# evo-design/evo

Measured on AMD Instinct MI355X. Metric: nucleotides/sec forward scoring, evo-1 7B, higher is better.
Workload: dtype bf16; 1 GPU; evo-1-8k-base scoring, batch 8 x 8,192 nt per GPU (BASELINE configs[1]); batch_per_gpu=8, nt=8192, parallelism=single GPU

## Files before the change

### evo_amd/csrc/gemm.hip

```cpp
#include <stdlib.h>
#include "common.h"
#include "../../include/evo_mi355x.h"

#define GBM 256
#define GBN 256
#define GBK 64
#define G_ROW (GBK * 2)
#define G_SLAB (GBM * G_ROW)
#define G_NSLOT 5
#define G_NP 4

typedef uint32_t g_u32x4 __attribute__((ext_vector_type(4)));

#define G_VMCNT(N) asm volatile("s_waitcnt vmcnt(%0)" ::"n"(N) : "memory")
#define G_BARRIER() asm volatile("s_barrier" ::: "memory")

struct GemmArgs {
    const unsigned char* x; const unsigned char* w; const uint16_t* bias; const uint16_t* res; uint16_t* y;
    int64_t M; int N; int K;
    int tiles_n; int n_tiles; int tiles_m; int group_m;
    const float* rs = nullptr;
    float* ss = nullptr;
    int64_t ss_ld = 0;
    int64_t w_rows = 0;
    int tm_tiles = 0, row_skip = 0;
};

template <bool BIAS, bool RES>
__global__ __launch_bounds__(512, 1) void gemm_bf16_kernel(GemmArgs a) {
    __shared__ __attribute__((aligned(16))) unsigned char smem[G_NSLOT * G_SLAB];
    const int tid = threadIdx.x;
    const int lane = tid & 63;
    const int wave = __builtin_amdgcn_readfirstlane(tid >> 6);
    const int half = lane >> 5;
    const int l31 = lane & 31;
    const int wm = wave >> 2, wn = wave & 3;

    int tile;
    {
        const int bid = blockIdx.x, nt = a.n_tiles;
        const int q = nt >> 3, r = nt & 7, xcd = bid & 7, slot = bid >> 3;
        tile = (xcd < r ? xcd * (q + 1) : r * (q + 1) + (xcd - r) * q) + slot;
    }
    int tm, tn;
    {
        const int per_group = a.group_m * a.tiles_n;
        const int grp = tile / per_group, in_grp = tile - grp * per_group;
        const int first_m = grp * a.group_m;
        const int gsz = a.tiles_m - first_m < a.group_m ? a.tiles_m - first_m : a.group_m;
        tn = in_grp / gsz;
        tm = first_m + in_grp - tn * gsz;
    }
    const int64_t m0 = (int64_t)tm * GBM;
    const int n0 = tn * GBN;
    const int64_t kb = (int64_t)a.K * 2;
    const int nk = a.K / GBK;

    const unsigned char* srcx[G_NP];
    const unsigned char* srcw[G_NP];
#pragma unroll
    for (int jj = 0; jj < G_NP; ++jj) {
        const int pos = (wave + 8 * jj) * 1024 + 16 * lane;
        const int r = pos / G_ROW;
        const int col = ((((pos - r * G_ROW) >> 4) ^ (r >> 1)) & 7) * 16;
        int64_t m = m0 + r;
        if (m > a.M - 1) m = a.M - 1;
        srcx[jj] = a.x + m * kb + col;
        srcw[jj] = a.w + (int64_t)(n0 + r) * kb + col;
    }
    const uint32_t lds0 = (uint32_t)(uintptr_t)(__attribute__((address_space(3))) unsigned char*)smem;
    const uint32_t lds_dma = lds0 + wave * 1024;
#define G_DMA(SRC, H, JJ)                                                                                     \
    asm volatile("s_mov_b32 m0, %0\n\ts_nop 0\n\tglobal_load_lds_dwordx4 %1, off"                             \
                 ::"s"(lds_dma + ((H) % G_NSLOT) * G_SLAB + (JJ) * 8192),                                     \
                   "v"((SRC)[JJ] + (int64_t)(((H) >> 1) < nk ? ((H) >> 1) : nk - 1) * (GBK * 2)) : "memory", "m0")

    uint32_t x_rd[4], w_rd[4];
#pragma unroll
    for (int ks = 0; ks < 4; ++ks) {
        const int xr = wm * 128 + l31, wr = wn * 64 + l31;
        x_rd[ks] = lds0 + (uint32_t)(xr * G_ROW + (((2 * ks + half) ^ (xr >> 1)) & 7) * 16);
        w_rd[ks] = lds0 + (uint32_t)(wr * G_ROW + (((2 * ks + half) ^ (wr >> 1)) & 7) * 16);
    }

    f32x16_t acc[2][4];
#pragma unroll
    for (int i = 0; i < 2; ++i)
#pragma unroll
        for (int j = 0; j < 4; ++j)
#pragma unroll
            for (int r = 0; r < 16; ++r) acc[i][j][r] = 0.f;
    g_u32x4 wf[2][2], xf[2][4];

#define G_DSR(DST, ADDR, OFF) asm volatile("ds_read_b128 %0, %1 offset:%2" : "=v"(DST) : "v"(ADDR), "n"(OFF))
#define G_READ(XO, WO, KS, BUF)                                                                               \
    {                                                                                                         \
        const uint32_t wa_ = (WO) + w_rd[KS], xa_ = (XO) + x_rd[KS];                                          \
        G_DSR(wf[BUF][0], wa_, 0); G_DSR(wf[BUF][1], wa_, 32 * G_ROW);                                        \
        G_DSR(xf[BUF][0], xa_, 0); G_DSR(xf[BUF][1], xa_, 32 * G_ROW);                                        \
        G_DSR(xf[BUF][2], xa_, 64 * G_ROW); G_DSR(xf[BUF][3], xa_, 96 * G_ROW);                               \
    }
#define G_LGKM(N, BUF)                                                                                        \
    asm volatile("s_waitcnt lgkmcnt(%6)" : "+v"(wf[BUF][0]), "+v"(wf[BUF][1]), "+v"(xf[BUF][0]), "+v"(xf[BUF][1]), \
                 "+v"(xf[BUF][2]), "+v"(xf[BUF][3]) : "n"(N))
#define G_MFMA(I, J, BUF)                                                                                     \
    acc[I][J] = __builtin_amdgcn_mfma_f32_32x32x16_bf16(__builtin_bit_cast(bf16x8_t, wf[BUF][I]),             \
                                                        __builtin_bit_cast(bf16x8_t, xf[BUF][J]), acc[I][J], 0, 0, 0)
#define G_DMA_PIN(SRC, H, JJ)                                                                                 \
    {                                                                                                         \
        __builtin_amdgcn_sched_barrier(0);                                                                    \
        G_DMA(SRC, H, JJ);                                                                                    \
        __builtin_amdgcn_sched_barrier(0);                                                                    \
    }
#define G_MMA_DMA(BUF, SRC, H, JA, JB, JC, JD)                                                                \
    {                                                                                                         \
        G_MFMA(0, 0, BUF); G_MFMA(0, 1, BUF);                                                                 \
        if ((JA) >= 0) G_DMA_PIN(SRC, H, (JA) < 0 ? 0 : (JA));                                                    \
        G_MFMA(0, 2, BUF); G_MFMA(0, 3, BUF);                                                                 \
        if ((JB) >= 0) G_DMA_PIN(SRC, H, (JB) < 0 ? 0 : (JB));                                                    \
        G_MFMA(1, 0, BUF); G_MFMA(1, 1, BUF);                                                                 \
        if ((JC) >= 0) G_DMA_PIN(SRC, H, (JC) < 0 ? 0 : (JC));                                                    \
        G_MFMA(1, 2, BUF); G_MFMA(1, 3, BUF);                                                                 \
        if ((JD) >= 0) G_DMA_PIN(SRC, H, (JD) < 0 ? 0 : (JD));                                                    \
    }

#pragma unroll
    for (int jj = 0; jj < G_NP; ++jj) G_DMA(srcx, 0, jj);
#pragma unroll
    for (int jj = 0; jj < G_NP; ++jj) G_DMA(srcw, 1, jj);
    if (nk > 1) {
#pragma unroll
        for (int jj = 0; jj < G_NP; ++jj) G_DMA(srcx, 2, jj);
#pragma unroll
        for (int jj = 0; jj < G_NP; ++jj) G_DMA(srcw, 3, jj);
        G_VMCNT(2 * G_NP);
    } else {
        G_VMCNT(0);
    }
    G_BARRIER();
    G_READ(0, G_SLAB, 0, 0);
    for (int k = 0; k + 1 < nk; ++k) {
        const uint32_t xo = ((2 * k) % G_NSLOT) * G_SLAB, wo = ((2 * k + 1) % G_NSLOT) * G_SLAB;
        G_READ(xo, wo, 1, 1);
        G_LGKM(6, 0);
        __builtin_amdgcn_sched_barrier(0);
        G_MMA_DMA(0, srcx, 2 * k + 4, -1, 0, -1, 1);
        __builtin_amdgcn_sched_barrier(0);
        G_READ(xo, wo, 2, 0);
        G_LGKM(6, 1);
        __builtin_amdgcn_sched_barrier(0);
        G_MMA_DMA(1, srcx, 2 * k + 4, -1, 2, -1, 3);
        __builtin_amdgcn_sched_barrier(0);
        G_READ(xo, wo, 3, 1);
        G_LGKM(6, 0);
        __builtin_amdgcn_sched_barrier(0);
        G_MMA_DMA(0, srcx, 0, -1, -1, -1, -1);
        __builtin_amdgcn_sched_barrier(0);
        G_LGKM(0, 1);
        G_VMCNT(G_NP);
        G_BARRIER();
        G_READ(((2 * k + 2) % G_NSLOT) * G_SLAB, ((2 * k + 3) % G_NSLOT) * G_SLAB, 0, 0);
        __builtin_amdgcn_sched_barrier(0);
        G_MMA_DMA(1, srcw, 2 * k + 5, 0, 1, 2, 3);
        __builtin_amdgcn_sched_barrier(0);
    }
    {
        const int k = nk - 1;
        const uint32_t xo = ((2 * k) % G_NSLOT) * G_SLAB, wo = ((2 * k + 1) % G_NSLOT) * G_SLAB;
        G_READ(xo, wo, 1, 1);
        G_LGKM(6, 0);
        G_MMA_DMA(0, srcx, 0, -1, -1, -1, -1);
        G_READ(xo, wo, 2, 0);
        G_LGKM(6, 1);
        G_MMA_DMA(1, srcx, 0, -1, -1, -1, -1);
        G_READ(xo, wo, 3, 1);
        G_LGKM(6, 0);
        G_MMA_DMA(0, srcx, 0, -1, -1, -1, -1);
        G_LGKM(0, 1);
        G_MMA_DMA(1, srcx, 0, -1, -1, -1, -1);
        G_VMCNT(0);
    }

    G_BARRIER();
    {
        constexpr int PITCH = 144;
        unsigned char* tr = smem + wave * (128 * PITCH);
        const int rsub = lane >> 3, cseg = lane & 7;
        const int nseg = n0 + wn * 64 + cseg * 8;
        if (RES) {
#pragma unroll 4
            for (int it = 0; it < 16; ++it) {
                const int row = it * 8 + rsub;
                const int64_t m = m0 + wm * 128 + row;
                uint4 r = make_uint4(0, 0, 0, 0);
                if (m < a.M) r = *(const uint4*)(a.res + m * a.N + nseg);
                *(uint4*)(tr + row * PITCH + cseg * 16) = r;
            }
        }
        asm volatile("" ::: "memory");
        uint2 bpk[2][4];
        if (BIAS) {
#pragma unroll
            for (int i = 0; i < 2; ++i)
#pragma unroll
                for (int g = 0; g < 4; ++g) bpk[i][g] = *(const uint2*)(a.bias + n0 + wn * 64 + i * 32 + 8 * g + 4 * half);
        }
#pragma unroll
        for (int j = 0; j < 4; ++j)
#pragma unroll
            for (int i = 0; i < 2; ++i)
#pragma unroll
                for (int g = 0; g < 4; ++g) {
                    unsigned char* cell = tr + (j * 32 + l31) * PITCH + (i * 32 + 8 * g + 4 * half) * 2;
                    float v[4] = {acc[i][j][4 * g], acc[i][j][4 * g + 1], acc[i][j][4 * g + 2], acc[i][j][4 * g + 3]};
                    if (BIAS) {
                        v[0] += bf_lo(bpk[i][g].x); v[1] += bf_hi(bpk[i][g].x);
                        v[2] += bf_lo(bpk[i][g].y); v[3] += bf_hi(bpk[i][g].y);
                    }
                    if (RES) {
                        const uint2 r = *(const uint2*)cell;
                        v[0] += bf_lo(r.x); v[1] += bf_hi(r.x); v[2] += bf_lo(r.y); v[3] += bf_hi(r.y);
                    }
                    uint2 o;
                    o.x = pack_bf2(v[0], v[1]);
                    o.y = pack_bf2(v[2], v[3]);
                    *(uint2*)cell = o;
                }
        asm volatile("" ::: "memory");
#pragma unroll 4
        for (int it = 0; it < 16; ++it) {
            const int row = it * 8 + rsub;
            const int64_t m = m0 + wm * 128 + row;
            const uint4 o = *(const uint4*)(tr + row * PITCH + cseg * 16);
            if (m < a.M) *(uint4*)(a.y + m * a.N + nseg) = o;
        }
    }
}


#ifndef GR_DGAP
#define GR_DGAP 8
#endif
#ifndef GE_ORDER
#define GE_ORDER 1
#endif
#ifndef GE_FULL
#define GE_FULL 1
#endif
static_assert(!GE_FULL || GE_ORDER == 1, "GE_FULL pairs the strips of GE_ORDER 1");
#if GE_ORDER == 0
#define GE_B(U) ((U) >> 3)
#define GE_J(U) ((U) & 7)
#else
#define GE_B(U) ((U) & 3)
#define GE_J(U) ((U) >> 2)
#endif

#ifndef GE_STPOL_ID
#define GE_STPOL_ID 0
#endif
#if GE_STPOL_ID == 1
#define GE_STPOL " nt"
#elif GE_STPOL_ID == 2
#define GE_STPOL " sc1"
#elif GE_STPOL_ID == 3
#define GE_STPOL " sc0 sc1"
#else
#define GE_STPOL ""
#endif
#ifndef GR_MIDB
#define GR_MIDB 1
#endif
#ifndef GR_PAD
#define GR_PAD 0
#endif
#ifndef GR_ALIGN
#define GR_ALIGN 0
#endif
#ifndef GR_PROFILE
#define GR_PROFILE 0
#endif

template <bool BIAS, bool RES, int MODE, bool XB = false, int NF = 0>
__global__ __launch_bounds__(256, 1) void gemmr_bf16_kernel(GemmArgs a) {
    constexpr bool STATS = (NF & 1) != 0, SCALE = (NF & 2) != 0;
    static_assert(!STATS || (RES && MODE == 0), "the statistic rides on the launches that write the residual stream");
    static_assert(!SCALE || !RES, "the row factor belongs to the launches that read the normalised stream");
    constexpr uint32_t XSTEP = XB ? 16384u : (uint32_t)(GBK * 2);
    __shared__ __attribute__((aligned(16))) unsigned char smem[G_NSLOT * G_SLAB];
    const int tid = threadIdx.x;
    const int lane = tid & 63;
    const int wave = __builtin_amdgcn_readfirstlane(tid >> 6);
    const int wm = wave >> 1, wn = wave & 1;
    const uint32_t kb = (uint32_t)a.K * 2;
    const int nk = a.K / GBK;

    int t_first, t_step, n_my;
    {
        const int bid = blockIdx.x, per = gridDim.x >> 3;
        const int xcd = bid & 7, slot = bid >> 3;
        const int q = a.n_tiles >> 3, r = a.n_tiles & 7;
        const int xs = xcd < r ? xcd * (q + 1) : r * (q + 1) + (xcd - r) * q;
        const int xn = q + (xcd < r ? 1 : 0);
        t_first = xs + slot;
        t_step = per;
        n_my = slot < xn ? (xn - slot + per - 1) / per : 0;
    }
    if (n_my == 0) return;
    auto tile_origin = [&](int tile, int64_t& m0, int& n0) {
        if constexpr (MODE == 3) {
            const int per_group = a.group_m * a.tiles_m;
            const int grp = tile / per_group, in_grp = tile - grp * per_group;
            const int first_n = grp * a.group_m;
            const int gsz = a.tiles_n - first_n < a.group_m ? a.tiles_n - first_n : a.group_m;
            const int tm = in_grp / gsz;
            m0 = (int64_t)tm * GBM;
            n0 = (first_n + in_grp - tm * gsz) * GBN;
            return;
        }
        const int per_group = a.group_m * a.tiles_n;
        const int grp = tile / per_group, in_grp = tile - grp * per_group;
        const int first_m = grp * a.group_m;
        const int gsz = a.tiles_m - first_m < a.group_m ? a.tiles_m - first_m : a.group_m;
        const int tn = in_grp / gsz;
        m0 = (int64_t)(first_m + in_grp - tn * gsz) * GBM;
        n0 = tn * GBN;
    };

    auto src_row = [&](int n0) -> uint32_t {
        if constexpr (MODE == 3 && SCALE) return (uint32_t)n0 + (uint32_t)((n0 / GBN) / a.tm_tiles) * (uint32_t)a.row_skip;
        else return (uint32_t)n0;
    };

    const int r0 = 8 * wave + (lane >> 3);
    const uint32_t xs_ = (uint32_t)(((lane & 7) ^ r0) & 7);
    const uint32_t voff0 = XB ? (uint32_t)r0 * 32u + (xs_ >> 1) * 4096u + (xs_ & 1) * 16u
                              : (uint32_t)r0 * kb + xs_ * 16;
    const uint32_t row32 = 32u * kb;
    uint32_t voff[8], wvoff[8];
    const int wrow = 8 * ((r0 >> 2) & 3) + 4 * ((r0 >> 4) & 1) + (r0 & 3);
    const uint32_t wvoff0 = (uint32_t)wrow * kb + (uint32_t)((((lane & 7) ^ r0) & 7) * 16);
#pragma unroll
    for (int jj = 0; jj < 8; ++jj) {
        voff[jj] = XB ? voff0 + (uint32_t)(jj & 3) * 1024u + (uint32_t)(jj >> 2) * 128u * kb : voff0 + jj * row32;
        wvoff[jj] = wvoff0 + jj * row32;
    }
    const uint64_t xa64 = (uint64_t)a.x, wa64 = (uint64_t)a.w;
    const g_u32x4 rx = {(uint32_t)xa64, (uint32_t)(xa64 >> 32) & 0xffffu,
                        (uint32_t)((XB ? (a.M + 127) / 128 * 128 : a.M) * (int64_t)kb), 0x00020000u};
    const g_u32x4 rw = {(uint32_t)wa64, (uint32_t)(wa64 >> 32) & 0xffffu, (uint32_t)((MODE == 3 && SCALE ? a.w_rows : (int64_t)a.N) * kb), 0x00020000u};
    const uint32_t lds0 = (uint32_t)(uintptr_t)(__attribute__((address_space(3))) unsigned char*)smem;
    const uint32_t lds_dma = lds0 + wave * 1024;

    int f_i = 0, f_k = 0;
    uint32_t fxs, fws;
    {
        int64_t m0; int n0;
        tile_origin(t_first, m0, n0);
        fxs = (uint32_t)(m0 * kb);
        fws = src_row(n0) * kb;
    }
    auto fetch_advance = [&]() {
        if (f_k + 1 < nk) { ++f_k; fxs += XSTEP; fws += GBK * 2; }
        else if (f_i + 1 < n_my) {
            ++f_i; f_k = 0;
            int64_t m0; int n0;
            tile_origin(t_first + f_i * t_step, m0, n0);
            fxs = (uint32_t)(m0 * kb);
            fws = src_row(n0) * kb;
        }
    };
    uint32_t nx0 = 0, nw0 = 0, nfxs = 0, nfws = 0, fxp = 0, fwp = 0;
    int f_rem = 0;
    auto next_tile_origin = [&]() {
        if (f_i + 1 < n_my) {
            int64_t m0; int n0;
            tile_origin(t_first + (f_i + 1) * t_step, m0, n0);
            nx0 = (uint32_t)(m0 * kb);
            nw0 = src_row(n0) * kb;
        }
    };
#define GD_M0(V) asm volatile("s_mov_b32 m0, %0" ::"s"(V) : "memory", "m0")
#ifndef GR_ABL
#define GR_ABL 0
#endif
#define GD_DMAX(JJ) asm volatile("buffer_load_dwordx4 %0, %1, %2 offen lds" ::"v"(voff[JJ]), "s"(rx), "s"(fxs) : "memory")
#define GD_DMAW(JJ) asm volatile("buffer_load_dwordx4 %0, %1, %2 offen lds" ::"v"(wvoff[JJ]), "s"(rw), "s"(fws) : "memory")

    const int l15 = lane & 15, lq = lane >> 4;
    uint32_t x_rd[2], w_rd[2];
#pragma unroll
    for (int kh = 0; kh < 2; ++kh) {
        const int xr = wm * 128 + l15, wr = wn * 128 + l15;
        x_rd[kh] = lds0 + (uint32_t)(xr * G_ROW + (((4 * kh + lq) ^ xr) & 7) * 16);
        w_rd[kh] = lds0 + (uint32_t)(wr * G_ROW + (((4 * kh + lq) ^ wr) & 7) * 16);
    }

    const int ldy = MODE == 3 ? GBN : a.N;
    const uint32_t ep_voff = (uint32_t)((wm * 128 + l15) * ldy + wn * 128 + 8 * lq) * 2u;
    const int ep_rows16 = 16 * ldy * 2;
    const uint32_t ep_voff_f = (uint32_t)((wm * 128 + (l15 & 7)) * ldy + wn * 128 + 8 * lq + 32 * (l15 >> 3)) * 2u;
    const uint32_t ep_boff = (uint32_t)(wn * 128 + 8 * lq) * 2u;
    const uint32_t ep_rboff = (uint32_t)(wm * 128 + l15) * 2u;
    const uint32_t ep_rsoff = (uint32_t)(wm * 128 + l15) * 4u;
    const uint32_t ep_rsoff3 = (uint32_t)(wn * 128 + 8 * lq) * 4u;
    const int ep_gn = a.N >> 1;
    const uint32_t ep_voff_g = (uint32_t)((wm * 128 + (l15 & 7)) * ep_gn + wn * 64 + 8 * lq + 32 * (l15 >> 3)) * 2u;
    const int ep_grows16 = 16 * ep_gn * 2;
    f32x4_t acc[8][8];
#define GR_ZERO1(I, J) { _Pragma("unroll") for (int r_ = 0; r_ < 4; ++r_) acc[I][J][r_] = 0.f; asm volatile("" : "+a"(acc[I][J])); }
#define GR_ZERO() _Pragma("unroll") for (int i = 0; i < 8; ++i) _Pragma("unroll") for (int j = 0; j < 8; ++j) GR_ZERO1(i, j)
    GR_ZERO();
    asm volatile("s_nop 7" ::: "memory");
    g_u32x4 wf[2][8], xf[2][8];

#define GR_LGKM(N, BUF)                                                                                       \
    asm volatile("s_waitcnt lgkmcnt(%16)" : "+v"(wf[BUF][0]), "+v"(wf[BUF][1]), "+v"(wf[BUF][2]), "+v"(wf[BUF][3]), \
                 "+v"(wf[BUF][4]), "+v"(wf[BUF][5]), "+v"(wf[BUF][6]), "+v"(wf[BUF][7]),                      \
                 "+v"(xf[BUF][0]), "+v"(xf[BUF][1]), "+v"(xf[BUF][2]), "+v"(xf[BUF][3]),                      \
                 "+v"(xf[BUF][4]), "+v"(xf[BUF][5]), "+v"(xf[BUF][6]), "+v"(xf[BUF][7]) : "n"(N))
#define GR_MFMA(I, J, BUF)                                                                                    \
    asm volatile("v_mfma_f32_16x16x32_bf16 %0, %1, %2, %0" : "+a"(acc[I][J]) : "v"(wf[BUF][I]), "v"(xf[BUF][J]))
#define GR_RD1(XO, WO, KH, BUF, Q)                                                                            \
    { if ((Q) < 8) G_DSR(xf[BUF][(Q) & 7], (XO) + x_rd[KH], ((Q) & 7) * 16 * G_ROW);                          \
      else G_DSR(wf[BUF][(Q) & 7], (WO) + w_rd[KH], ((Q) & 7) * 16 * G_ROW); }
#define GR_GAP(G, RXO, RWO, RKH, RBUF)                                                                        \
    {                                                                                                         \
        __builtin_amdgcn_sched_barrier(0);                                                                    \
        constexpr int g_ = (G), s_ = g_ & 63;                                                                 \
         \
         \
        if constexpr (g_ == 64 && GR_MIDB) { G_VMCNT(8); if (!(GR_ABL & 2)) G_BARRIER(); }                    \
        if constexpr ((s_ & 1) == 0 && s_ < 32 && !(GR_ABL & 8)) { GR_RD1(RXO, RWO, RKH, RBUF, s_ >> 1); }    \
        if constexpr (g_ < 64 && s_ < 8 * GR_DGAP && (s_ % GR_DGAP) == 1 && !(GR_ABL & 16)) GD_M0(fxl + (s_ / GR_DGAP) * 4096);        \
        if constexpr (g_ < 64 && s_ < 8 * GR_DGAP && (s_ % GR_DGAP) == GR_DGAP / 2 + 1 && !(GR_ABL & 1)) GD_DMAX(s_ / GR_DGAP);       \
        if constexpr (g_ >= 64 && s_ < 8 * GR_DGAP && (s_ % GR_DGAP) == 1 && !(GR_ABL & 16)) GD_M0(fwl + (s_ / GR_DGAP) * 4096);       \
        if constexpr (g_ >= 64 && s_ < 8 * GR_DGAP && (s_ % GR_DGAP) == GR_DGAP / 2 + 1 && !(GR_ABL & 1)) GD_DMAW(s_ / GR_DGAP);      \
         \
         \
        if constexpr (g_ == 67) { fxp = fxs + XSTEP; fwp = fws + GBK * 2; GS_PIN2(fxp, fwp); }              \
        if constexpr (g_ == 71) { f_rem -= 1; GS_PIN1(f_rem); }                                               \
        if constexpr (g_ == 75) { nfxs = f_rem == 0 ? nx0 : fxp; GS_PIN1(nfxs); }                             \
        if constexpr (g_ == 87) { nfws = f_rem == 0 ? nw0 : fwp; GS_PIN1(nfws); }                             \
        if constexpr (g_ == 110) { c_k -= 1; GS_PIN1(c_k); }                                                  \
        if constexpr (g_ == 91) { const bool z_ = f_rem == 0; f_rem = z_ ? nk : f_rem; f_i += z_ ? 1 : 0; GS_PIN2(f_rem, f_i); } \
        if constexpr (g_ == 83) { fxs = nfxs; GS_PIN1(fxs); }                                                 \
         \
        if constexpr (g_ == 96) { r_t0 = xo; xo = nxo; GS_PIN2(r_t0, xo); }                                   \
        if constexpr (g_ == 98) { r_t1 = wo; wo = nwo; GS_PIN2(r_t1, wo); }                                   \
        if constexpr (g_ == 100) { nxo = fxo; nwo = r_t0; GS_PIN2(nxo, nwo); }                                \
        if constexpr (g_ == 102) { fxo = r_t1; fxl = lds_dma + r_t1; GS_PIN2(fxo, fxl); }                     \
        if constexpr (g_ == 126) { fws = nfws; fwl = lds_dma + xo; GS_PIN2(fws, fwl); }                       \
        __builtin_amdgcn_sched_barrier(0);                                                                    \
    }
#define GR_ROW8(SS, I, BUF, RXO, RWO, RKH, RBUF)                                                              \
    {                                                                                                         \
        GR_MFMA(I, 0, BUF); GR_GAP(64 * (SS) + 8 * (I) + 0, RXO, RWO, RKH, RBUF); GR_MFMA(I, 1, BUF); GR_GAP(64 * (SS) + 8 * (I) + 1, RXO, RWO, RKH, RBUF); \
        GR_MFMA(I, 2, BUF); GR_GAP(64 * (SS) + 8 * (I) + 2, RXO, RWO, RKH, RBUF); GR_MFMA(I, 3, BUF); GR_GAP(64 * (SS) + 8 * (I) + 3, RXO, RWO, RKH, RBUF); \
        GR_MFMA(I, 4, BUF); GR_GAP(64 * (SS) + 8 * (I) + 4, RXO, RWO, RKH, RBUF); GR_MFMA(I, 5, BUF); GR_GAP(64 * (SS) + 8 * (I) + 5, RXO, RWO, RKH, RBUF); \
        GR_MFMA(I, 6, BUF); GR_GAP(64 * (SS) + 8 * (I) + 6, RXO, RWO, RKH, RBUF); GR_MFMA(I, 7, BUF); GR_GAP(64 * (SS) + 8 * (I) + 7, RXO, RWO, RKH, RBUF); \
    }
#define GR_SUB(SS, BUF, RXO, RWO, RKH, RBUF)                                                                  \
    {                                                                                                         \
        GR_ROW8(SS, 0, BUF, RXO, RWO, RKH, RBUF); GR_ROW8(SS, 1, BUF, RXO, RWO, RKH, RBUF);                   \
        GR_ROW8(SS, 2, BUF, RXO, RWO, RKH, RBUF); GR_ROW8(SS, 3, BUF, RXO, RWO, RKH, RBUF);                   \
        GR_ROW8(SS, 4, BUF, RXO, RWO, RKH, RBUF); GR_ROW8(SS, 5, BUF, RXO, RWO, RKH, RBUF);                   \
        GR_ROW8(SS, 6, BUF, RXO, RWO, RKH, RBUF); GR_ROW8(SS, 7, BUF, RXO, RWO, RKH, RBUF);                   \
    }
#define GS_PIN1(A) asm volatile("" : "+s"(A))
#define GS_PIN2(A, B) asm volatile("" : "+s"(A), "+s"(B))

#pragma unroll
    for (int jj = 0; jj < 8; ++jj) { GD_M0(lds_dma + 0 * G_SLAB + jj * 4096); asm volatile("s_nop 0"); GD_DMAX(jj); }
#pragma unroll
    for (int jj = 0; jj < 8; ++jj) { GD_M0(lds_dma + 1 * G_SLAB + jj * 4096); asm volatile("s_nop 0"); GD_DMAW(jj); }
    fetch_advance();
#pragma unroll
    for (int jj = 0; jj < 8; ++jj) { GD_M0(lds_dma + 2 * G_SLAB + jj * 4096); asm volatile("s_nop 0"); GD_DMAX(jj); }
#pragma unroll
    for (int jj = 0; jj < 8; ++jj) { GD_M0(lds_dma + 3 * G_SLAB + jj * 4096); asm volatile("s_nop 0"); GD_DMAW(jj); }
    fetch_advance();
    f_rem = nk - f_k;
    next_tile_origin();
    G_VMCNT(16);
    G_BARRIER();
    {
        const uint32_t x0_ = 0, w0_ = G_SLAB;
#pragma unroll
        for (int q = 0; q < 16; ++q) GR_RD1(x0_, w0_, 0, 0, q);
    }

#if GR_PROFILE
    const bool prof = blockIdx.x == 0 && wave == 0;
    uint64_t tp[12] = {0, 0, 0, 0, 0, 0, 0, 0, 0, 0, 0, 0}, tl = __builtin_readcyclecounter();
#define GR_STAMP(K) if (prof) { const uint64_t n_ = __builtin_readcyclecounter(); tp[K] += n_ - tl; tl = n_; }
#else
#define GR_STAMP(K)
#endif
    uint32_t xo = 0, wo = G_SLAB, nxo = 2 * G_SLAB, nwo = 3 * G_SLAB, fxo = 4 * G_SLAB;
    uint32_t fxl = lds_dma + 4 * G_SLAB, fwl = lds_dma, r_t0 = 0, r_t1 = 0;
#if GR_PAD
    asm volatile(".rept %0\n\ts_nop 0\n\t.endr" :: "n"(GR_PAD));
#endif
#if GR_ALIGN
    asm volatile(".p2align %0" :: "n"(GR_ALIGN));
#endif
    for (int c_i = 0; c_i < n_my; ++c_i) {
#define GR_KSTEP()                                                                                            \
        {                                                                                                     \
            GR_LGKM(0, 0);                                                                                    \
            GR_STAMP(5);                                                                                      \
            GR_SUB(0, 0, xo, wo, 1, 1);                                                                       \
            GR_STAMP(0);                                                                                      \
            GR_LGKM(0, 1);                                        \
            GR_STAMP(1);                                                                                      \
            if (!GR_MIDB) { G_VMCNT(8); GR_STAMP(2); if (!(GR_ABL & 2)) G_BARRIER(); }                        \
            GR_STAMP(6);                                                                                      \
            GR_SUB(1, 1, nxo, nwo, 0, 0);                                                                     \
            GR_STAMP(3);                                                                                      \
        }
        for (int c_k = nk; c_k != 0;) GR_KSTEP();
        {
            asm volatile("s_nop 7\n\ts_nop 7" ::: "memory");
            int64_t m0; int n0;
            tile_origin(t_first + c_i * t_step, m0, n0);
            GR_STAMP(7);
            if constexpr (MODE == 1) {
                const int rows_ok = a.M - m0 < GBM ? (int)(a.M - m0) : GBM;
                const uint64_t y64 = (uint64_t)(a.y + m0 * ep_gn);
                const g_u32x4 yd = {(uint32_t)y64, (uint32_t)(y64 >> 32) & 0xffffu, (uint32_t)(rows_ok * ep_gn * 2), 0x00020000u};
                g_u32x4 ost[8], gq[2];
                float rsj[8];
                if constexpr (SCALE) {
#pragma unroll
                    for (int j = 0; j < 8; ++j)
                        asm volatile("global_load_dword %0, %1, %2" : "=v"(rsj[j]) : "v"(ep_rsoff), "s"(a.rs + m0 + 16 * j) : "memory");
                    asm volatile("s_waitcnt vmcnt(0)" : "+v"(rsj[0]), "+v"(rsj[1]), "+v"(rsj[2]), "+v"(rsj[3]), "+v"(rsj[4]), "+v"(rsj[5]),
                                 "+v"(rsj[6]), "+v"(rsj[7]) :: "memory");
                }
#pragma unroll
                for (int j = 0; j < 8; ++j) {
#pragma unroll
                    for (int pp = 0; pp < 2; ++pp) {
                        __builtin_amdgcn_sched_barrier(0);
                        float z1[8], z2[8];
#pragma unroll
                        for (int r = 0; r < 4; ++r) {
                            asm volatile("v_accvgpr_read_b32 %0, %1" : "=v"(z1[r]) : "a"(acc[4 * pp][j][r]));
                            asm volatile("v_accvgpr_read_b32 %0, %1" : "=v"(z1[4 + r]) : "a"(acc[4 * pp + 1][j][r]));
                            asm volatile("v_accvgpr_read_b32 %0, %1" : "=v"(z2[r]) : "a"(acc[4 * pp + 2][j][r]));
                            asm volatile("v_accvgpr_read_b32 %0, %1" : "=v"(z2[4 + r]) : "a"(acc[4 * pp + 3][j][r]));
                        }
                        GR_ZERO1(4 * pp, j); GR_ZERO1(4 * pp + 1, j); GR_ZERO1(4 * pp + 2, j); GR_ZERO1(4 * pp + 3, j);
                        if constexpr (SCALE) {
#pragma unroll
                            for (int e = 0; e < 8; ++e) { z1[e] *= rsj[j]; z2[e] *= rsj[j]; }
                        }
#pragma unroll
                        for (int e = 0; e < 8; e += 2) {
                            const uint32_t u1 = pack_bf2(z1[e], z1[e + 1]), u2 = pack_bf2(z2[e], z2[e + 1]);
                            const f32x2_t uu = {bf_lo(u1), bf_hi(u1)}, ww = {bf_lo(u2), bf_hi(u2)};
                            const f32x2_t oo = gelu_gate2(uu, ww);
                            gq[pp][e >> 1] = pack_bf2(oo[0], oo[1]);
                        }
                    }
                    const bool low = l15 < 8;
                    g_u32x4 &s1 = ost[(2 * j) & 7], &s2 = ost[(2 * j + 1) & 7];
#pragma unroll
                    for (int d = 0; d < 4; ++d) {
                        const uint32_t give = low ? gq[1][d] : gq[0][d];
                        const uint32_t recv = (uint32_t)__builtin_amdgcn_update_dpp(0, (int)give, 0x128, 0xf, 0xf, false);
                        s1[d] = low ? gq[0][d] : recv;
                        s2[d] = low ? recv : gq[1][d];
                    }
                    const int so = n0 + j * ep_grows16;
                    asm volatile("buffer_store_dwordx4 %0, %1, %2, %3 offen" GE_STPOL :: "v"(s1), "v"(ep_voff_g), "s"(yd), "s"(so) : "memory");
                    asm volatile("buffer_store_dwordx4 %0, %1, %2, %3 offen" GE_STPOL :: "v"(s2), "v"(ep_voff_g), "s"(yd), "s"(so + ep_grows16 / 2) : "memory");
                    if (j >= 3) { asm volatile("" :: "v"(ost[(2 * j + 2) & 7])); asm volatile("" :: "v"(ost[(2 * j + 3) & 7])); }
                }
                __builtin_amdgcn_sched_barrier(0);
#pragma unroll
                for (int k = 0; k < 8; ++k) asm volatile("" :: "v"(ost[k]));
                GR_STAMP(8);
            } else {
            const int rows_ok = a.M - m0 < GBM ? (int)(a.M - m0) : GBM;
            const uint64_t y64 = (uint64_t)(MODE == 3 ? a.y + ((int64_t)(n0 / GBN) * a.M + m0) * GBN : a.y + m0 * a.N);
            const uint64_t r64 = (uint64_t)((RES ? a.res : a.y) + m0 * a.N);
            const g_u32x4 yd = {(uint32_t)y64, (uint32_t)(y64 >> 32) & 0xffffu, (uint32_t)(rows_ok * ldy * 2), 0x00020000u};
            const g_u32x4 rd = {(uint32_t)r64, (uint32_t)(r64 >> 32) & 0xffffu, RES ? (uint32_t)(rows_ok * a.N * 2) : 0u, 0x00020000u};
#define GE_SOFF(U) ((MODE == 3 ? 0 : n0 * 2) + 64 * GE_B(U) + GE_J(U) * ep_rows16)
#define GE_NR 6
#define GE_LOAD(U) asm volatile("buffer_load_dwordx4 %0, %1, %2, %3 offen" : "=v"(rr[(U) % GE_NR]) : "v"(ep_voff), "s"(rd), "s"(GE_SOFF(U)) : "memory")
            g_u32x4 rr[GE_NR], bq[4], ost[8], o_even;
            uint32_t rbq[8];
            float rsj[8];
            g_u32x4 rsq[4][2];
            if constexpr (SCALE && MODE == 0) {
#pragma unroll
                for (int j = 0; j < 8; ++j)
                    asm volatile("global_load_dword %0, %1, %2" : "=v"(rsj[j]) : "v"(ep_rsoff), "s"(a.rs + m0 + 16 * j) : "memory");
                asm volatile("s_waitcnt vmcnt(0)" : "+v"(rsj[0]), "+v"(rsj[1]), "+v"(rsj[2]), "+v"(rsj[3]), "+v"(rsj[4]), "+v"(rsj[5]),
                             "+v"(rsj[6]), "+v"(rsj[7]) :: "memory");
            }
            if constexpr (SCALE && MODE == 3) {
                const float* rs0 = a.rs + src_row(n0);
#pragma unroll
                for (int b = 0; b < 4; ++b) {
                    asm volatile("global_load_dwordx4 %0, %1, %2" : "=v"(rsq[b][0]) : "v"(ep_rsoff3), "s"(rs0 + b * 32) : "memory");
                    asm volatile("global_load_dwordx4 %0, %1, %2" : "=v"(rsq[b][1]) : "v"(ep_rsoff3), "s"(rs0 + b * 32 + 4) : "memory");
                }
                asm volatile("s_waitcnt vmcnt(0)" : "+v"(rsq[0][0]), "+v"(rsq[0][1]), "+v"(rsq[1][0]), "+v"(rsq[1][1]), "+v"(rsq[2][0]),
                             "+v"(rsq[2][1]), "+v"(rsq[3][0]), "+v"(rsq[3][1]) :: "memory");
            }
            float ssq = 0.f, sst[4];
            if (BIAS && MODE != 3) {
#pragma unroll
                for (int b = 0; b < 4; ++b)
                    asm volatile("global_load_dwordx4 %0, %1, %2" : "=v"(bq[b]) : "v"(ep_boff), "s"(a.bias + n0 + b * 32) : "memory");
            }
            if (BIAS && MODE == 3) {
#pragma unroll
                for (int j = 0; j < 8; ++j)
                    asm volatile("global_load_ushort %0, %1, %2" : "=v"(rbq[j]) : "v"(ep_rboff), "s"(a.bias + m0 + 16 * j) : "memory");
                asm volatile("s_waitcnt vmcnt(0)" : "+v"(rbq[0]), "+v"(rbq[1]), "+v"(rbq[2]), "+v"(rbq[3]), "+v"(rbq[4]), "+v"(rbq[5]),
                             "+v"(rbq[6]), "+v"(rbq[7]) :: "memory");
            }
            if (RES) {
#pragma unroll
                for (int u = 0; u < GE_NR; ++u) GE_LOAD(u);
            }
            if (BIAS && !RES && MODE != 3) asm volatile("s_waitcnt vmcnt(0)" : "+v"(bq[0]), "+v"(bq[1]), "+v"(bq[2]), "+v"(bq[3]) :: "memory");
#pragma unroll
            for (int u = 0; u < 32; ++u) {
                const int b = GE_B(u), j = GE_J(u);
                __builtin_amdgcn_sched_barrier(0);
                if (RES) {
                    if (u + GE_NR <= 32) asm volatile("s_waitcnt vmcnt(%5)" : "+v"(rr[u % GE_NR]), "+v"(bq[0]), "+v"(bq[1]), "+v"(bq[2]), "+v"(bq[3]) : "n"(GE_NR - 1) : "memory");
                    else asm volatile("s_waitcnt vmcnt(0)" : "+v"(rr[u % GE_NR]) :: "memory");
                }
                float v[8];
#pragma unroll
                for (int r = 0; r < 4; ++r) {
                    asm volatile("v_accvgpr_read_b32 %0, %1" : "=v"(v[r]) : "a"(acc[2 * b][j][r]));
                    asm volatile("v_accvgpr_read_b32 %0, %1" : "=v"(v[4 + r]) : "a"(acc[2 * b + 1][j][r]));
                }
                GR_ZERO1(2 * b, j); GR_ZERO1(2 * b + 1, j);
                if constexpr (SCALE && MODE == 0) {
#pragma unroll
                    for (int e = 0; e < 8; ++e) v[e] *= rsj[j];
                }
                if constexpr (SCALE && MODE == 3) {
#pragma unroll
                    for (int e = 0; e < 8; ++e) v[e] *= __uint_as_float(rsq[b][e >> 2][e & 3]);
                }
                if (BIAS && MODE != 3) {
                    v[0] += bf_lo(bq[b][0]); v[1] += bf_hi(bq[b][0]); v[2] += bf_lo(bq[b][1]); v[3] += bf_hi(bq[b][1]);
                    v[4] += bf_lo(bq[b][2]); v[5] += bf_hi(bq[b][2]); v[6] += bf_lo(bq[b][3]); v[7] += bf_hi(bq[b][3]);
                }
                if (BIAS && MODE == 3) {
                    const float rb = bf_lo(rbq[j]);
#pragma unroll
                    for (int e = 0; e < 8; ++e) v[e] += rb;
                }
                if (RES) {
                    const g_u32x4 r = rr[u % GE_NR];
                    v[0] += bf_lo(r[0]); v[1] += bf_hi(r[0]); v[2] += bf_lo(r[1]); v[3] += bf_hi(r[1]);
                    v[4] += bf_lo(r[2]); v[5] += bf_hi(r[2]); v[6] += bf_lo(r[3]); v[7] += bf_hi(r[3]);
                }
                g_u32x4 o;
                o[0] = pack_bf2(v[0], v[1]); o[1] = pack_bf2(v[2], v[3]); o[2] = pack_bf2(v[4], v[5]); o[3] = pack_bf2(v[6], v[7]);
                if constexpr (STATS) {
                    static_assert(GE_ORDER == 1, "the statistic closes an m tile at b == 3");
#pragma unroll
                    for (int d = 0; d < 4; ++d) {
                        const float lo_ = bf_lo(o[d]), hi_ = bf_hi(o[d]);
                        ssq = fmaf(lo_, lo_, ssq);
                        ssq = fmaf(hi_, hi_, ssq);
                    }
                    if (b == 3) {
                        float t_ = ssq + __uint_as_float((uint32_t)__builtin_amdgcn_ds_swizzle((int)__float_as_uint(ssq), 0x401f));
                        t_ += __shfl_xor(t_, 32);
                        sst[j & 3] = t_;
                        const float* sp_ = a.ss + ((int64_t)(n0 / 128 + wn) * a.ss_ld + m0 + 16 * j);
                        asm volatile("global_store_dword %0, %1, %2" :: "v"(ep_rsoff), "v"(sst[j & 3]), "s"(sp_) : "memory");
                        ssq = 0.f;
                    }
                }
#if GE_FULL
                if ((u & 1) == 0) o_even = o;
                else {
                    const bool low = l15 < 8;
                    g_u32x4 &s1 = ost[(u - 1) & 7], &s2 = ost[u & 7];
#pragma unroll
                    for (int d = 0; d < 4; ++d) {
                        const uint32_t give = low ? o[d] : o_even[d];
                        const uint32_t recv = (uint32_t)__builtin_amdgcn_update_dpp(0, (int)give, 0x128, 0xf, 0xf, false);
                        s1[d] = low ? o_even[d] : recv;
                        s2[d] = low ? recv : o[d];
                    }
                    asm volatile("buffer_store_dwordx4 %0, %1, %2, %3 offen" GE_STPOL :: "v"(s1), "v"(ep_voff_f), "s"(yd), "s"(GE_SOFF(u - 1)) : "memory");
                    asm volatile("buffer_store_dwordx4 %0, %1, %2, %3 offen" GE_STPOL :: "v"(s2), "v"(ep_voff_f), "s"(yd), "s"(GE_SOFF(u - 1) + ep_rows16 / 2) : "memory");
                    if (u >= 7) { asm volatile("" :: "v"(ost[(u + 1) & 7])); asm volatile("" :: "v"(ost[(u + 2) & 7])); }
                }
#else
                ost[u & 7] = o;
                asm volatile("buffer_store_dwordx4 %0, %1, %2, %3 offen" GE_STPOL :: "v"(ost[u & 7]), "v"(ep_voff), "s"(yd), "s"(GE_SOFF(u)) : "memory");
                if (u >= 7) asm volatile("" :: "v"(ost[(u + 1) & 7]));
#endif
                if (RES && u + GE_NR < 32) GE_LOAD(u + GE_NR);
            }
            __builtin_amdgcn_sched_barrier(0);
#pragma unroll
            for (int k = 0; k < 8; ++k) asm volatile("" :: "v"(ost[k]));
            if constexpr (STATS) asm volatile("" :: "v"(sst[0]), "v"(sst[1]), "v"(sst[2]), "v"(sst[3]));
            GR_STAMP(8);
#undef GE_LOAD
#undef GE_NR
#undef GE_SOFF
            }
            next_tile_origin();
            GR_STAMP(9);
            asm volatile("s_nop 7" ::: "memory");
            GR_STAMP(4);
        }
    }
    G_VMCNT(0);
#if GR_PROFILE
    if (prof && lane == 0) {
        for (int k = 0; k < 12; ++k) ((float*)a.y)[k] = (float)tp[k];
        ((float*)a.y)[12] = (float)(n_my * nk);
        ((float*)a.y)[13] = (float)n_my;
    }
#endif
}

extern "C" int evo_linear_mfma_bf16(const void* x, const void* w, const void* bias, const void* residual, void* y,
                                    int64_t M, int64_t N, int64_t K, void* stream) {
    return evo_linear_mfma_nf_bf16(x, w, bias, residual, y, nullptr, nullptr, 0, M, N, K, stream);
}

extern "C" int evo_linear_mfma_nf_bf16(const void* x, const void* w, const void* bias, const void* residual, void* y,
                                       const float* row_scale, float* sumsq, int64_t ss_ld, int64_t M, int64_t N, int64_t K, void* stream) {
    if (M <= 0 || N <= 0 || K <= 0 || N % GBN != 0 || K % GBK != 0 || N > 0x7fffffff / 2) return -1;
    if ((row_scale && (residual || sumsq)) || (sumsq && (!residual || ss_ld < (M + GBM - 1) / GBM * GBM))) return -1;
    if ((row_scale || sumsq) && !(K >= 2 * GBK && M * K * 2 < 0xffffffffll && N * K * 2 < 0xffffffffll)) return -1;
    GemmArgs a;
    a.rs = row_scale; a.ss = sumsq; a.ss_ld = ss_ld;
    a.x = (const unsigned char*)x; a.w = (const unsigned char*)w; a.bias = (const uint16_t*)bias;
    a.res = (const uint16_t*)residual; a.y = (uint16_t*)y;
    a.M = M; a.N = (int)N; a.K = (int)K;
    a.tiles_n = (int)(N / GBN);
    a.tiles_m = (int)((M + GBM - 1) / GBM);
    const int group_m = (a.tiles_n >= 32 ? 8 : 4);
    a.group_m = group_m;
    const int64_t tiles = ((M + GBM - 1) / GBM) * a.tiles_n;
    if (tiles > 0x7fffffff) return -1;
    a.n_tiles = (int)tiles;
    const dim3 grid((unsigned)tiles), block(512);
    hipStream_t st = (hipStream_t)stream;
    static const int form = [] { const char* e = getenv("EVO_GEMM_FORM"); return e ? atoi(e) : 1; }();
    if ((row_scale || sumsq) && form != 1) return -1;
    if (form == 1 && K >= 2 * GBK && M * K * 2 < 0xffffffffll && N * K * 2 < 0xffffffffll) {
        static const int n_cu = [] {
            int dev = 0, n = 256;
            if (hipGetDevice(&dev) == hipSuccess) (void)hipDeviceGetAttribute(&n, hipDeviceAttributeMultiprocessorCount, dev);
            n &= ~7;
            return n < 8 ? 8 : n;
        }();
        const dim3 gridp((unsigned)n_cu), block4(256);
        if (row_scale) {
            if (bias) hipLaunchKernelGGL((gemmr_bf16_kernel<true, false, 0, false, 2>), gridp, block4, 0, st, a);
            else hipLaunchKernelGGL((gemmr_bf16_kernel<false, false, 0, false, 2>), gridp, block4, 0, st, a);
            return evo_launch_status();
        }
        if (sumsq) {
            if (bias) hipLaunchKernelGGL((gemmr_bf16_kernel<true, true, 0, false, 1>), gridp, block4, 0, st, a);
            else hipLaunchKernelGGL((gemmr_bf16_kernel<false, true, 0, false, 1>), gridp, block4, 0, st, a);
            return evo_launch_status();
        }
        if (bias && residual) hipLaunchKernelGGL((gemmr_bf16_kernel<true, true, 0>), gridp, block4, 0, st, a);
        else if (bias) hipLaunchKernelGGL((gemmr_bf16_kernel<true, false, 0>), gridp, block4, 0, st, a);
        else if (residual) hipLaunchKernelGGL((gemmr_bf16_kernel<false, true, 0>), gridp, block4, 0, st, a);
        else hipLaunchKernelGGL((gemmr_bf16_kernel<false, false, 0>), gridp, block4, 0, st, a);
        return evo_launch_status();
    }
    if (bias && residual) hipLaunchKernelGGL((gemm_bf16_kernel<true, true>), grid, block, 0, st, a);
    else if (bias) hipLaunchKernelGGL((gemm_bf16_kernel<true, false>), grid, block, 0, st, a);
    else if (residual) hipLaunchKernelGGL((gemm_bf16_kernel<false, true>), grid, block, 0, st, a);
    else hipLaunchKernelGGL((gemm_bf16_kernel<false, false>), grid, block, 0, st, a);
    return evo_launch_status();
}

extern "C" int evo_linear_xblk_mfma_bf16(const void* x_blk, const void* w, const void* bias, const void* residual, void* y,
                                         int64_t M, int64_t N, int64_t K, void* stream) {
    return evo_linear_xblk_mfma_nf_bf16(x_blk, w, bias, residual, y, nullptr, 0, M, N, K, stream);
}

extern "C" int evo_linear_xblk_mfma_nf_bf16(const void* x_blk, const void* w, const void* bias, const void* residual, void* y,
                                            float* sumsq, int64_t ss_ld, int64_t M, int64_t N, int64_t K, void* stream) {
    if (sumsq && (!residual || ss_ld < M)) return -1;
    if (M <= 0 || M % GBM != 0 || N <= 0 || K <= 0 || N % GBN != 0 || K % GBK != 0 || K < 2 * GBK || N > 0x7fffffff / 2) return -1;
    if (M * K * 2 >= 0xffffffffll || N * K * 2 >= 0xffffffffll) return -1;
    GemmArgs a;
    a.x = (const unsigned char*)x_blk; a.w = (const unsigned char*)w; a.bias = (const uint16_t*)bias;
    a.res = (const uint16_t*)residual; a.y = (uint16_t*)y;
    a.ss = sumsq; a.ss_ld = ss_ld;
    a.M = M; a.N = (int)N; a.K = (int)K;
    a.tiles_n = (int)(N / GBN);
    a.tiles_m = (int)(M / GBM);
    a.group_m = a.tiles_n >= 32 ? 8 : 4;
    const int64_t tiles = (M / GBM) * a.tiles_n;
    if (tiles > 0x7fffffff) return -1;
    a.n_tiles = (int)tiles;
    static const int n_cu = [] {
        int dev = 0, n = 256;
        if (hipGetDevice(&dev) == hipSuccess) (void)hipDeviceGetAttribute(&n, hipDeviceAttributeMultiprocessorCount, dev);
        n &= ~7;
        return n < 8 ? 8 : n;
    }();
    const dim3 gridp((unsigned)n_cu), block4(256);
    if (sumsq) {
        if (bias) hipLaunchKernelGGL((gemmr_bf16_kernel<true, true, 0, true, 1>), gridp, block4, 0, (hipStream_t)stream, a);
        else hipLaunchKernelGGL((gemmr_bf16_kernel<false, true, 0, true, 1>), gridp, block4, 0, (hipStream_t)stream, a);
        return evo_launch_status();
    }
    if (bias && residual) hipLaunchKernelGGL((gemmr_bf16_kernel<true, true, 0, true>), gridp, block4, 0, (hipStream_t)stream, a);
    else if (residual) hipLaunchKernelGGL((gemmr_bf16_kernel<false, true, 0, true>), gridp, block4, 0, (hipStream_t)stream, a);
    else if (bias) hipLaunchKernelGGL((gemmr_bf16_kernel<true, false, 0, true>), gridp, block4, 0, (hipStream_t)stream, a);
    else hipLaunchKernelGGL((gemmr_bf16_kernel<false, false, 0, true>), gridp, block4, 0, (hipStream_t)stream, a);
    return evo_launch_status();
}

extern "C" int evo_mlp_gate_mfma_bf16(const void* x, const void* w12g, void* a_out, int64_t M, int64_t I, int64_t K, void* stream) {
    return evo_mlp_gate_mfma_nf_bf16(x, nullptr, w12g, a_out, M, I, K, stream);
}

extern "C" int evo_mlp_gate_mfma_nf_bf16(const void* x, const float* row_scale, const void* w12g, void* a_out, int64_t M, int64_t I, int64_t K,
                                         void* stream) {
    const int64_t N = 2 * I;
    if (M <= 0 || I <= 0 || K <= 0 || N % GBN != 0 || K % GBK != 0 || K < 2 * GBK || N > 0x7fffffff / 2) return -1;
    if (M * K * 2 >= 0xffffffffll || N * K * 2 >= 0xffffffffll) return -1;
    GemmArgs a;
    a.x = (const unsigned char*)x; a.w = (const unsigned char*)w12g; a.bias = nullptr; a.res = nullptr; a.y = (uint16_t*)a_out;
    a.rs = row_scale;
    a.M = M; a.N = (int)N; a.K = (int)K;
    a.tiles_n = (int)(N / GBN);
    a.tiles_m = (int)((M + GBM - 1) / GBM);
    a.group_m = (a.tiles_n >= 32 ? 8 : 4);
    const int64_t tiles = (int64_t)a.tiles_m * a.tiles_n;
    if (tiles > 0x7fffffff) return -1;
    a.n_tiles = (int)tiles;
    static const int n_cu = [] {
        int dev = 0, n = 256;
        if (hipGetDevice(&dev) == hipSuccess) (void)hipDeviceGetAttribute(&n, hipDeviceAttributeMultiprocessorCount, dev);
        n &= ~7;
        return n < 8 ? 8 : n;
    }();
    if (row_scale) hipLaunchKernelGGL((gemmr_bf16_kernel<false, false, 1, false, 2>), dim3((unsigned)n_cu), dim3(256), 0, (hipStream_t)stream, a);
    else hipLaunchKernelGGL((gemmr_bf16_kernel<false, false, 1>), dim3((unsigned)n_cu), dim3(256), 0, (hipStream_t)stream, a);
    return evo_launch_status();
}

extern "C" int evo_linear_t_mfma_bf16(const void* x, const void* w, const void* bias, void* zt, int64_t Mp, int64_t N, int64_t K,
                                      void* stream) {
    return evo_linear_t_mfma_nf_bf16(x, nullptr, w, bias, zt, Mp, N, K, Mp, Mp, 0, stream);
}

extern "C" int evo_linear_t_mfma_nf_bf16(const void* x, const float* row_scale, const void* w, const void* bias, void* zt, int64_t Mp, int64_t N,
                                         int64_t K, int64_t x_rows, int64_t Tm, int64_t row_skip, void* stream) {
    if (row_scale) {
        if (Tm <= 0 || Tm % GBN != 0 || Mp % Tm != 0 || row_skip < 0 || row_skip > 0x7fff || x_rows < Mp + (Mp / Tm - 1) * row_skip
            || x_rows * K * 2 >= 0xffffffffll) return -1;
    } else if (x_rows != Mp || Tm != Mp || row_skip != 0) return -1;
    if (Mp <= 0 || N <= 0 || K <= 0 || Mp % GBN != 0 || N % GBM != 0 || K % GBK != 0 || K < 2 * GBK || Mp > 0x7fffffff / 2) return -1;
    if (Mp * K * 2 >= 0xffffffffll || N * K * 2 >= 0xffffffffll) return -1;
    GemmArgs a;
    a.x = (const unsigned char*)w; a.w = (const unsigned char*)x; a.bias = (const uint16_t*)bias; a.res = nullptr; a.y = (uint16_t*)zt;
    a.M = N; a.N = (int)Mp; a.K = (int)K;
    a.rs = row_scale; a.w_rows = x_rows; a.tm_tiles = (int)(Tm / GBN); a.row_skip = (int)row_skip;
    a.tiles_n = (int)(Mp / GBN);
    a.tiles_m = (int)(N / GBM);
    a.group_m = (a.tiles_m >= 32 ? 8 : 4);
    const int64_t tiles = (int64_t)a.tiles_m * a.tiles_n;
    if (tiles > 0x7fffffff) return -1;
    a.n_tiles = (int)tiles;
    static const int n_cu = [] {
        int dev = 0, n = 256;
        if (hipGetDevice(&dev) == hipSuccess) (void)hipDeviceGetAttribute(&n, hipDeviceAttributeMultiprocessorCount, dev);
        n &= ~7;
        return n < 8 ? 8 : n;
    }();
    if (row_scale) {
        if (bias) hipLaunchKernelGGL((gemmr_bf16_kernel<true, false, 3, false, 2>), dim3((unsigned)n_cu), dim3(256), 0, (hipStream_t)stream, a);
        else hipLaunchKernelGGL((gemmr_bf16_kernel<false, false, 3, false, 2>), dim3((unsigned)n_cu), dim3(256), 0, (hipStream_t)stream, a);
        return evo_launch_status();
    }
    if (bias) hipLaunchKernelGGL((gemmr_bf16_kernel<true, false, 3>), dim3((unsigned)n_cu), dim3(256), 0, (hipStream_t)stream, a);
    else hipLaunchKernelGGL((gemmr_bf16_kernel<false, false, 3>), dim3((unsigned)n_cu), dim3(256), 0, (hipStream_t)stream, a);
    return evo_launch_status();
}
```

Measured before the change: 111,100 nt/s.

## Carry GEMM epilogue stores into the next tile's first k-steps

For launches without a residual, the last 16 output store pairs of each tile's epilogue are held in registers and issued one per k-step during the next tile's main loop. This overlaps the global-store tail with MFMA work instead of stalling at the end of each tile. The vmcnt waits are adjusted to account for the extra in-flight stores. The cost is 16 extra vector registers of carried data and more complex unrolled code, which may raise register pressure or disturb the tuned schedule.

```diff
diff --git a/evo_amd/csrc/gemm.hip b/evo_amd/csrc/gemm.hip
--- a/evo_amd/csrc/gemm.hip
+++ b/evo_amd/csrc/gemm.hip
@@ -280,6 +280,11 @@
 #ifndef GR_PROFILE
 #define GR_PROFILE 0
 #endif
+#ifndef GR_CARRY
+#define GR_CARRY 1
+#endif
+#define GR_CK 16
+static_assert(!GR_CARRY || GE_FULL, "the carried stores are the whole-line pairs of GE_FULL");
 
 template <bool BIAS, bool RES, int MODE, bool XB = false, int NF = 0>
 __global__ __launch_bounds__(256, 1) void gemmr_bf16_kernel(GemmArgs a) {
@@ -287,6 +292,8 @@
     static_assert(!STATS || (RES && MODE == 0), "the statistic rides on the launches that write the residual stream");
     static_assert(!SCALE || !RES, "the row factor belongs to the launches that read the normalised stream");
     constexpr uint32_t XSTEP = XB ? 16384u : (uint32_t)(GBK * 2);
+    constexpr bool CARRY = GR_CARRY && !RES;
+    constexpr int GR_NB = MODE == 1 ? 0 : 16;
     __shared__ __attribute__((aligned(16))) unsigned char smem[G_NSLOT * G_SLAB];
     const int tid = threadIdx.x;
     const int lane = tid & 63;
@@ -407,6 +414,16 @@
     const int ep_gn = a.N >> 1;
     const uint32_t ep_voff_g = (uint32_t)((wm * 128 + (l15 & 7)) * ep_gn + wn * 64 + 8 * lq + 32 * (l15 >> 3)) * 2u;
     const int ep_grows16 = 16 * ep_gn * 2;
+    g_u32x4 cst[GR_CK], cyd = {0u, 0u, 0u, 0u};
+    int cso = 0;
+    const bool carry = CARRY && nk > GR_CK;
+    auto c_soff = [&](int t) -> int {
+        if constexpr (MODE == 1) return cso + t * (ep_grows16 / 2);
+        else return cso + 64 * (t & 2) + (4 + (t >> 2)) * ep_rows16 + (t & 1) * (ep_rows16 / 2);
+    };
+#define GR_CSTORE(T)                                                                                          \
+    asm volatile("buffer_store_dwordx4 %0, %1, %2, %3 offen" GE_STPOL                                         \
+                 :: "v"(cst[T]), "v"(MODE == 1 ? ep_voff_g : ep_voff_f), "s"(cyd), "s"(c_soff(T)) : "memory")
     f32x4_t acc[8][8];
 #define GR_ZERO1(I, J) { _Pragma("unroll") for (int r_ = 0; r_ < 4; ++r_) acc[I][J][r_] = 0.f; asm volatile("" : "+a"(acc[I][J])); }
 #define GR_ZERO() _Pragma("unroll") for (int i = 0; i < 8; ++i) _Pragma("unroll") for (int j = 0; j < 8; ++j) GR_ZERO1(i, j)
@@ -430,7 +447,11 @@
         constexpr int g_ = (G), s_ = g_ & 63;                                                                 \
          \
          \
-        if constexpr (g_ == 64 && GR_MIDB) { G_VMCNT(8); if (!(GR_ABL & 2)) G_BARRIER(); }                    \
+        if constexpr (g_ == 64 && GR_MIDB) { G_VMCNT(GR_VM); if (!(GR_ABL & 2)) G_BARRIER(); }                \
+         \
+         \
+        if constexpr (gr_kt >= 0 && gr_kt < GR_CK && g_ == 127) GR_CSTORE(gr_kt < 0 || gr_kt >= GR_CK ? 0 : gr_kt);       \
+        if constexpr (gr_kt >= 1 && g_ == 64) asm volatile("" :: "v"(cst[gr_kt < 1 ? 0 : gr_kt - 1]));                     \
         if constexpr ((s_ & 1) == 0 && s_ < 32 && !(GR_ABL & 8)) { GR_RD1(RXO, RWO, RKH, RBUF, s_ >> 1); }    \
         if constexpr (g_ < 64 && s_ < 8 * GR_DGAP && (s_ % GR_DGAP) == 1 && !(GR_ABL & 16)) GD_M0(fxl + (s_ / GR_DGAP) * 4096);        \
         if constexpr (g_ < 64 && s_ < 8 * GR_DGAP && (s_ % GR_DGAP) == GR_DGAP / 2 + 1 && !(GR_ABL & 1)) GD_DMAX(s_ / GR_DGAP);       \
@@ -505,21 +526,34 @@
 #if GR_ALIGN
     asm volatile(".p2align %0" :: "n"(GR_ALIGN));
 #endif
-    for (int c_i = 0; c_i < n_my; ++c_i) {
+    constexpr int gr_kt = -1;
+#define GR_VM (gr_kt < 0 ? 8 : gr_kt == 0 ? 8 + GR_NB : 9)
+#define GR_SID(K) (gr_kt < 0 ? (K) : 10)
 #define GR_KSTEP()                                                                                            \
         {                                                                                                     \
             GR_LGKM(0, 0);                                                                                    \
-            GR_STAMP(5);                                                                                      \
+            GR_STAMP(GR_SID(5));                                                                              \
             GR_SUB(0, 0, xo, wo, 1, 1);                                                                       \
-            GR_STAMP(0);                                                                                      \
+            GR_STAMP(GR_SID(0));                                                                              \
             GR_LGKM(0, 1);                                        \
-            GR_STAMP(1);                                                                                      \
-            if (!GR_MIDB) { G_VMCNT(8); GR_STAMP(2); if (!(GR_ABL & 2)) G_BARRIER(); }                        \
-            GR_STAMP(6);                                                                                      \
+            GR_STAMP(GR_SID(1));                                                                              \
+            if (!GR_MIDB) { G_VMCNT(GR_VM); GR_STAMP(GR_SID(2)); if (!(GR_ABL & 2)) G_BARRIER(); }            \
+            GR_STAMP(GR_SID(6));                                                                              \
             GR_SUB(1, 1, nxo, nwo, 0, 0);                                                                     \
-            GR_STAMP(3);                                                                                      \
-        }
-        for (int c_k = nk; c_k != 0;) GR_KSTEP();
+            GR_STAMP(GR_SID(3));                                                                              \
+        }
+#define GR_KSTEP_C(T) { constexpr int gr_kt = (T); GR_KSTEP(); }
+    for (int c_i = 0; c_i < n_my; ++c_i) {
+        int c_k = nk;
+        if constexpr (CARRY) {
+            if (carry && c_i > 0) {
+                GR_KSTEP_C(0); GR_KSTEP_C(1); GR_KSTEP_C(2); GR_KSTEP_C(3); GR_KSTEP_C(4); GR_KSTEP_C(5);
+                GR_KSTEP_C(6); GR_KSTEP_C(7); GR_KSTEP_C(8); GR_KSTEP_C(9); GR_KSTEP_C(10); GR_KSTEP_C(11);
+                GR_KSTEP_C(12); GR_KSTEP_C(13); GR_KSTEP_C(14); GR_KSTEP_C(15); GR_KSTEP_C(16);
+                static_assert(GR_CK == 16, "one carry k-step per carried store, and one behind the last");
+            }
+        }
+        for (; c_k != 0;) GR_KSTEP();
         {
             asm volatile("s_nop 7\n\ts_nop 7" ::: "memory");
             int64_t m0; int n0;
@@ -573,14 +607,22 @@
                         s1[d] = low ? gq[0][d] : recv;
                         s2[d] = low ? recv : gq[1][d];
                     }
+                    if constexpr (CARRY) {
+                        cst[2 * j] = s1; cst[2 * j + 1] = s2;
+                    } else {
                     const int so = n0 + j * ep_grows16;
                     asm volatile("buffer_store_dwordx4 %0, %1, %2, %3 offen" GE_STPOL :: "v"(s1), "v"(ep_voff_g), "s"(yd), "s"(so) : "memory");
                     asm volatile("buffer_store_dwordx4 %0, %1, %2, %3 offen" GE_STPOL :: "v"(s2), "v"(ep_voff_g), "s"(yd), "s"(so + ep_grows16 / 2) : "memory");
                     if (j >= 3) { asm volatile("" :: "v"(ost[(2 * j + 2) & 7])); asm volatile("" :: "v"(ost[(2 * j + 3) & 7])); }
+                    }
                 }
                 __builtin_amdgcn_sched_barrier(0);
-#pragma unroll
-                for (int k = 0; k < 8; ++k) asm volatile("" :: "v"(ost[k]));
+                if constexpr (!CARRY) {
+#pragma unroll
+                    for (int k = 0; k < 8; ++k) asm volatile("" :: "v"(ost[k]));
+                } else {
+                    cyd = yd; cso = n0;
+                }
                 GR_STAMP(8);
             } else {
             const int rows_ok = a.M - m0 < GBM ? (int)(a.M - m0) : GBM;
@@ -698,9 +740,13 @@
                         s1[d] = low ? o_even[d] : recv;
                         s2[d] = low ? recv : o[d];
                     }
+                    if (CARRY && u >= 16) {
+                        cst[u < 17 ? 0 : u - 17] = s1; cst[u < 16 ? 0 : u - 16] = s2;
+                    } else {
                     asm volatile("buffer_store_dwordx4 %0, %1, %2, %3 offen" GE_STPOL :: "v"(s1), "v"(ep_voff_f), "s"(yd), "s"(GE_SOFF(u - 1)) : "memory");
                     asm volatile("buffer_store_dwordx4 %0, %1, %2, %3 offen" GE_STPOL :: "v"(s2), "v"(ep_voff_f), "s"(yd), "s"(GE_SOFF(u - 1) + ep_rows16 / 2) : "memory");
                     if (u >= 7) { asm volatile("" :: "v"(ost[(u + 1) & 7])); asm volatile("" :: "v"(ost[(u + 2) & 7])); }
+                    }
                 }
 #else
                 ost[u & 7] = o;
@@ -713,11 +759,20 @@
 #pragma unroll
             for (int k = 0; k < 8; ++k) asm volatile("" :: "v"(ost[k]));
             if constexpr (STATS) asm volatile("" :: "v"(sst[0]), "v"(sst[1]), "v"(sst[2]), "v"(sst[3]));
+            if constexpr (CARRY) { cyd = yd; cso = MODE == 3 ? 0 : n0 * 2; }
             GR_STAMP(8);
 #undef GE_LOAD
 #undef GE_NR
 #undef GE_SOFF
             }
+            if constexpr (CARRY) {
+                if (!carry || c_i + 1 == n_my) {
+                    __builtin_amdgcn_sched_barrier(0);
+                    GR_CSTORE(0); GR_CSTORE(1); GR_CSTORE(2); GR_CSTORE(3); GR_CSTORE(4); GR_CSTORE(5); GR_CSTORE(6); GR_CSTORE(7);
+                    GR_CSTORE(8); GR_CSTORE(9); GR_CSTORE(10); GR_CSTORE(11); GR_CSTORE(12); GR_CSTORE(13); GR_CSTORE(14); GR_CSTORE(15);
+                    __builtin_amdgcn_sched_barrier(0);
+                }
+            }
             next_tile_origin();
             GR_STAMP(9);
             asm volatile("s_nop 7" ::: "memory");
@@ -728,6 +783,7 @@
 #if GR_PROFILE
     if (prof && lane == 0) {
         for (int k = 0; k < 12; ++k) ((float*)a.y)[k] = (float)tp[k];
+        ((float*)a.y)[11] = (float)(carry ? (n_my - 1) * (GR_CK + 1) : 0);
         ((float*)a.y)[12] = (float)(n_my * nk);
         ((float*)a.y)[13] = (float)n_my;
     }
```

After: 111,400 nt/s, median of 6. No clear change (+0.3%).
